# ZhendongS/Physics-Informed-Neural-Network-for-Explainable-Fault-Diagnosis-in-Fuel-Cells

Hardware: AMD Instinct MI355X
Metric: pinn_train_samples_per_s (higher is better)
Workload: dtype f32 (split-operand matrix products on the 16-bit matrix cores, f32 accumulate, fp32-matmul accuracy: 2 fp16 parts / 3 MFMAs per product in forward, backward and weight gradients); 1 GPU; BASELINE configs[1]: 1000000 synthetic rows x 8 features per GPU, PINN [8,256,256,256,1] + variance head, step = train_dnn (fwd+NLL+bwd+wgrad+allreduce+Adam) + one iteration of each of the 5 physics stages; rows_per_gpu=1000000, global_rows=1000000, parallelism=dp1, precision=f32x6, backend=none (single process), world_size=1

## Files before the change

### physics-informed-neural-network-for-explainable-fault-diagnosis-in-fuel-cells_amd/csrc/pinn_residuals.hip

```cpp
#include <hip/hip_runtime.h>
#include <math.h>
#include "../../include/pinn_hip.h"

namespace {

constexpr int kThreads = 256;
constexpr int kMaxBlocks = 1024;

struct AffineDev {
  double x_min[8];
  double x_scale[8];
  double y_min, y_scale;
  float vn_scale, vn_min;
};

__device__ __forceinline__ float denorm(float v, double mn, double sc) {
  float t = (float)((double)v - mn);
  return (float)((double)t / sc);
}

__device__ __forceinline__ float clamp_min_t(float x, float lo) { return x != x ? x : fmaxf(x, lo); }
__device__ __forceinline__ float clamp_t(float x, float lo, float hi) { return x != x ? x : fminf(fmaxf(x, lo), hi); }

__device__ __forceinline__ double wave_sum(double v) {
#pragma unroll
  for (int off = 32; off > 0; off >>= 1) v += __shfl_down(v, off, 64);
  return v;
}

struct LamDev {
  float l1, l2, l3, lT1, lT3, lT5, lH1, lH2, lH3, lO1, lO2, lO3, P_H2O;
};
__device__ __forceinline__ LamDev load_lambdas(const float* __restrict__ lambdas) {
  LamDev L;
  L.l1 = lambdas[PINN_L1]; L.l2 = lambdas[PINN_L2]; L.l3 = lambdas[PINN_L3];
  L.lT1 = lambdas[PINN_LT1]; L.lT3 = lambdas[PINN_LT3]; L.lT5 = lambdas[PINN_LT5];
  L.lH1 = lambdas[PINN_LH1]; L.lH2 = lambdas[PINN_LH2]; L.lH3 = lambdas[PINN_LH3];
  L.lO1 = lambdas[PINN_LO1]; L.lO2 = lambdas[PINN_LO2]; L.lO3 = lambdas[PINN_LO3];
  const float Tc = 55.0f;
  const float xw = ((-2.1794f + 0.02953f * Tc) - 9.1837e-5f * (Tc * Tc)) + 1.4454e-7f * ((Tc * Tc) * Tc);
  L.P_H2O = powf(10.0f, xw);
  return L;
}

template <bool kCols>
__device__ __forceinline__ void row_terms(long long row, const float* __restrict__ x, const float* __restrict__ u, const float* __restrict__ y,
                                          const AffineDev& aff, const LamDev& L, unsigned flags, float* __restrict__ cols, long long ld,
                                          float (&acc)[PINN_NSUMS]) {
  const float l1 = L.l1, l2 = L.l2, l3 = L.l3, lT1 = L.lT1, lT3 = L.lT3, lT5 = L.lT5, lH1 = L.lH1, lH2 = L.lH2, lH3 = L.lH3;
  const float lO1 = L.lO1, lO2 = L.lO2, lO3 = L.lO3, P_H2O = L.P_H2O;

    const float4 xa = reinterpret_cast<const float4*>(x)[row * 2];
    const float4 xb = reinterpret_cast<const float4*>(x)[row * 2 + 1];
    const bool fV = flags & PINN_RES_V, fT = flags & PINN_RES_T, fH = flags & PINN_RES_H, fO = flags & PINN_RES_O;
    const float r0 = denorm(xa.x, aff.x_min[0], aff.x_scale[0]);
    const float r1 = fT ? denorm(xa.y, aff.x_min[1], aff.x_scale[1]) : 0.f;
    const float r2 = fT ? denorm(xa.z, aff.x_min[2], aff.x_scale[2]) : 0.f;
    const float r3 = fV ? denorm(xa.w, aff.x_min[3], aff.x_scale[3]) : 0.f;
    const float r4 = fV ? denorm(xb.x, aff.x_min[4], aff.x_scale[4]) : 0.f;
    const float r5 = (fV || fT) ? denorm(xb.y, aff.x_min[5], aff.x_scale[5]) : 0.f;
    const float r6 = fH ? denorm(xb.z, aff.x_min[6], aff.x_scale[6]) : 0.f;
    const float r7 = fO ? denorm(xb.w, aff.x_min[7], aff.x_scale[7]) : 0.f;
    const float yv = (y != nullptr) ? y[row] : 0.0f;

    const float i5 = r0 / 270.0f + 1e-5f;
    const float It = i5 * 270.0f;

    if (flags & PINN_RES_V) {
      const float un = u[row];
      const float Tk = r5 + 273.15f;
      const float P_H2 = r3 / 101.0f + 1.0f;
      const float P_air = r4 / 101.0f + 1.0f;
      const float Tk_p = powf(Tk, 1.334f);
      const float pp_H2 = 0.5f * (P_H2 / expf(1.653f * i5 / Tk_p) - P_H2O);
      const float pp_O2 = P_air / expf(4.192f * i5 / Tk_p) - P_H2O;
      const float RT = 8.314f * Tk;
      const float b = RT / 96485.0f;
      const float V_act = (-b) * logf(i5 / l2);
      const float V_ohm = -(i5 * l1);
      const float V_conc = (0.5f * b) * logf(1.0f - i5 / l3);
      const float E = 220170.0f / 192970.0f - (RT * logf(P_H2O / (pp_H2 * sqrtf(pp_O2)))) / 192970.0f;
      const float V_est = ((E + V_act) + V_ohm) + V_conc;
      const float V_out = denorm(un, aff.y_min, aff.y_scale) / 5.0f;
      const float f = V_est - V_out;
// ... 25 lines not shown
        cols[PINN_C_I * ld + row] = i5;
        cols[PINN_C_VOUT5 * ld + row] = V_out * 5.0f;
      }
    }

    if (flags & PINN_RES_T) {
      const float i6 = r0 / 270.0f + 1e-6f;
      const float mc = r1 + 1e-6f;
      const float It6 = i6 * 270.0f;
      const float T_pred = ((lT1 * It6 + lT3 * mc) + 0.5f * r2) + lT5;
      const float f = r5 - T_pred;
      acc[PINN_S_FT2] += f * f;
      acc[PINN_S_FT_D1] += f * (-It6);
      acc[PINN_S_FT_D3] += f * (-mc);
      acc[PINN_S_FT_D5] += -f;
      acc[PINN_S_FT_ABS] += fabsf(f);
      if (kCols) {
        cols[PINN_C_FT * ld + row] = f;
        cols[PINN_C_TPRED * ld + row] = T_pred;
        cols[PINN_C_TOUT * ld + row] = r5;
      }
    }

    if (flags & PINN_RES_H) {
      float Q = ((It / 192970.0f) * 5.0f) * 22.4f;
      Q = Q * 60.0f;
      Q = clamp_min_t(Q, 1e-8f);
      const bool lin = It <= lH3;
      const float tgt = lin ? (lH1 + lH2 * (It / 100.0f)) : (lH1 + lH2 * (lH3 / 100.0f));
      const float act = (r6 + 1e-6f) / Q;
      const float f = act - tgt;
      acc[PINN_S_FH2] += f * f;
      acc[PINN_S_FH_D1] += -f;
      acc[PINN_S_FH_D2] += f * (-(lin ? It / 100.0f : lH3 / 100.0f));
      acc[PINN_S_FH_D3] += f * (-(lin ? 0.0f : lH2 / 100.0f));
      acc[PINN_S_ACTH] += act;
      acc[PINN_S_TGTH] += tgt;
      if (kCols) {
        cols[PINN_C_FH * ld + row] = f;
        cols[PINN_C_ACTH * ld + row] = act;
        cols[PINN_C_TGTH * ld + row] = tgt;
        cols[PINN_C_ITOT * ld + row] = It;
      }
    }

    if (flags & PINN_RES_O) {
      float Q = ((It * 5.0f) / 385940.0f) * 22.4f;
      Q = Q * 60.0f;
      Q = clamp_min_t(Q, 1e-8f);
      const float thr = fabsf(lO3);
      const bool lin = It <= thr;
      const float raw = lin ? (lO1 + lO2 * (It / 100.0f)) : (lO1 + lO2 * (thr / 100.0f));
      const float tgt = clamp_t(raw, 1.05f, 15.0f);
      const float c = (raw >= 1.05f && raw <= 15.0f) ? 1.0f : 0.0f;
      const float o2 = (r7 + 1e-6f) * 0.21f;
      const float act = o2 / Q;
      const float f = (act - tgt) + clamp_min_t(1.0f - act, 0.0f) * 10.0f;
      const float sgn = (lO3 > 0.0f) ? 1.0f : ((lO3 < 0.0f) ? -1.0f : 0.0f);
      acc[PINN_S_FO2] += f * f;
      acc[PINN_S_FO_D1] += f * (-c);
      acc[PINN_S_FO_D2] += f * (-c * (lin ? It / 100.0f : thr / 100.0f));
      acc[PINN_S_FO_D3] += f * (-c * (lin ? 0.0f : lO2 * sgn / 100.0f));
      acc[PINN_S_ACTO] += act;
      acc[PINN_S_TGTO] += tgt;
      if (kCols) {
        cols[PINN_C_FO * ld + row] = f;
        cols[PINN_C_ACTO * ld + row] = act;
        cols[PINN_C_TGTO * ld + row] = tgt;
        cols[PINN_C_QO2 * ld + row] = Q;
        cols[PINN_C_O2FLOW * ld + row] = o2;
      }
    }
  }

struct SumRange { int lo, hi; };
constexpr SumRange live_sums(unsigned flags) {
  return flags == PINN_RES_V ? SumRange{PINN_S_FV2, PINN_S_YU2 + 1}
       : flags == PINN_RES_T ? SumRange{PINN_S_FT2, PINN_S_FT_ABS + 1}
       : flags == PINN_RES_H ? SumRange{PINN_S_FH2, PINN_S_TGTH + 1}
       : flags == PINN_RES_O ? SumRange{PINN_S_FO2, PINN_S_TGTO + 1}
                             : SumRange{0, PINN_NSUMS};
}

template <int kLo, int kHi, int kBlock>
__device__ __forceinline__ void block_partials(const float (&acc)[PINN_NSUMS], double* __restrict__ partials) {
  __shared__ double red[kBlock / 64][kHi - kLo];
  const int lane = threadIdx.x & 63, wave = threadIdx.x >> 6;
#pragma unroll
  for (int s = kLo; s < kHi; ++s) {
    const double w = wave_sum((double)acc[s]);
    if (lane == 0) red[wave][s - kLo] = w;
  }
  __syncthreads();
  if (threadIdx.x < kHi - kLo) {
    double t = 0.0;
#pragma unroll
    for (int w = 0; w < kBlock / 64; ++w) t += red[w][threadIdx.x];
    partials[(long long)blockIdx.x * PINN_NSUMS + kLo + threadIdx.x] = t;
  }
}

template <bool kCols, unsigned kFlags>
__global__ __launch_bounds__(kThreads) void residuals_kernel(
    const float* __restrict__ x, const float* __restrict__ u, const float* __restrict__ y, AffineDev aff,
    const float* __restrict__ lambdas, unsigned flags_rt, long long n_rows, float* __restrict__ cols, long long ld,
    double* __restrict__ partials) {
  const unsigned flags = kFlags ? kFlags : flags_rt;
  const LamDev L = load_lambdas(lambdas);
  float acc[PINN_NSUMS];
#pragma unroll
  for (int s = 0; s < PINN_NSUMS; ++s) acc[s] = 0.0f;

  const long long stride = (long long)gridDim.x * kThreads;
  for (long long row = (long long)blockIdx.x * kThreads + threadIdx.x; row < n_rows; row += stride)
    row_terms<kCols>(row, x, u, y, aff, L, flags, cols, ld, acc);

  if (partials == nullptr) return;
  block_partials<live_sums(kFlags).lo, live_sums(kFlags).hi, kThreads>(acc, partials);
}

__global__ __launch_bounds__(1024) void residuals_finalize(const double* __restrict__ partials, int n_blocks, int s_lo, int s_hi,
                                                           double* __restrict__ sums) {
  __shared__ double red[32][PINN_NSUMS + 1];
  const int s = threadIdx.x & 31, j = threadIdx.x >> 5;
  if (s >= s_lo && s < s_hi) {
    double v[kMaxBlocks / 32];
#pragma unroll
    for (int k = 0; k < kMaxBlocks / 32; ++k) {
      const int b = j + 32 * k;
      v[k] = b < n_blocks ? partials[(long long)b * PINN_NSUMS + s] : 0.0;
    }
    double t = 0.0;
#pragma unroll
    for (int k = 0; k < kMaxBlocks / 32; ++k) t += v[k];
    red[j][s] = t;
  }
  __syncthreads();
  if (threadIdx.x < PINN_NSUMS) {
    double r = 0.0;
    if (threadIdx.x >= s_lo && threadIdx.x < s_hi) {
#pragma unroll
      for (int k = 0; k < 32; ++k) r += red[k][threadIdx.x];
    }
    sums[threadIdx.x] = r;
  }
}

struct StageDef {
  int n;
  int idx[5];
  float lo[5], hi[5];
};

__device__ __forceinline__ void lambda_step_body(int stage, const double* sums, double inv_n, float vn_scale, float lr, double bc1, double bc2, float* lambdas,
                                 float* adam, float* loss_out) {
  StageDef d;
  float g[5];
  bool has_grad[5];
  float total = 0.f, physics = 0.f;
  if (stage == PINN_STAGE_LAMBDA_PM || stage == PINN_STAGE_LAMBDA_F) {
    d.n = 4;
    d.idx[0] = PINN_L1; d.idx[1] = PINN_L2; d.idx[2] = PINN_L3; d.idx[3] = PINN_L4;
    d.lo[0] = (float)(0.167 * 0.5); d.hi[0] = (float)(0.167 * 5);
    d.lo[1] = (float)(2.36e-6 * 0.1); d.hi[1] = (float)(2.36e-6 * 2.1);
    d.lo[2] = 2.0f; d.hi[2] = (float)(2.0 * 5.2);
    d.lo[3] = 0.1f; d.hi[3] = 10.0f;
    has_grad[3] = false; g[3] = 0.f;
    if (stage == PINN_STAGE_LAMBDA_F) {
      physics = (float)(sums[PINN_S_FV2] * inv_n);
      for (int k = 0; k < 3; ++k) { g[k] = (float)(2.0 * sums[PINN_S_FV_D1 + k] * inv_n); has_grad[k] = true; }
    } else {
      physics = (float)(sums[PINN_S_YV2] * inv_n);
      for (int k = 0; k < 3; ++k) {
        g[k] = (float)(-2.0 * 5.0 * (double)vn_scale * sums[PINN_S_YV_D1 + k] * inv_n);
        has_grad[k] = true;
      }
    }
    total = physics + (float)(sums[PINN_S_YU2] * inv_n);
  } else if (stage == PINN_STAGE_THERMAL) {
    d.n = 5;
    for (int k = 0; k < 5; ++k) { d.idx[k] = PINN_LT1 + k; d.lo[k] = -10000.f; d.hi[k] = 10000.f; has_grad[k] = false; g[k] = 0.f; }
    g[0] = (float)(2.0 * sums[PINN_S_FT_D1] * inv_n); has_grad[0] = true;
    g[2] = (float)(2.0 * sums[PINN_S_FT_D3] * inv_n); has_grad[2] = true;
    g[4] = (float)(2.0 * sums[PINN_S_FT_D5] * inv_n); has_grad[4] = true;
    total = physics = (float)(sums[PINN_S_FT2] * inv_n);
  } else if (stage == PINN_STAGE_HYDROGEN) {
    d.n = 4;
    for (int k = 0; k < 4; ++k) d.idx[k] = PINN_LH1 + k;
    d.lo[0] = 0.5f; d.hi[0] = 50.f; d.lo[1] = -20.f; d.hi[1] = 20.f; d.lo[2] = 50.f; d.hi[2] = 1000.f; d.lo[3] = 0.f; d.hi[3] = 20.f;
    for (int k = 0; k < 3; ++k) { g[k] = (float)(2.0 * sums[PINN_S_FH_D1 + k] * inv_n); has_grad[k] = true; }
    has_grad[3] = false; g[3] = 0.f;
    total = physics = (float)(sums[PINN_S_FH2] * inv_n);
  } else {
    d.n = 4;
    for (int k = 0; k < 4; ++k) d.idx[k] = PINN_LO1 + k;
    d.lo[0] = 1.5f; d.hi[0] = 8.f; d.lo[1] = -20.f; d.hi[1] = 20.f; d.lo[2] = 50.f; d.hi[2] = 1000.f; d.lo[3] = 0.f; d.hi[3] = 20.f;
    for (int k = 0; k < 3; ++k) { g[k] = (float)(2.0 * sums[PINN_S_FO_D1 + k] * inv_n); has_grad[k] = true; }
    has_grad[3] = false; g[3] = 0.f;
    total = physics = (float)(sums[PINN_S_FO2] * inv_n);
  }
  const float step_size = (float)((double)lr / bc1);
  const float bc2_sqrt = (float)sqrt(bc2);
#pragma unroll
  for (int k = 0; k < 5; ++k) {
    if (k >= d.n) break;
    const int id = d.idx[k];
    float p = lambdas[id];
    if (has_grad[k]) {
      float m = adam[id], v = adam[PINN_NLAMBDA + id];
      m = m * 0.9f + g[k] * 0.1f;
      v = v * 0.999f + (g[k] * g[k]) * 0.001f;
      const float denom = sqrtf(v) / bc2_sqrt + 1e-8f;
      p = p - step_size * (m / denom);
      adam[id] = m; adam[PINN_NLAMBDA + id] = v;
    }
    lambdas[id] = clamp_t(p, d.lo[k], d.hi[k]);
  }
  if (loss_out) { loss_out[0] = total; loss_out[1] = physics; }
}

__global__ void lambda_step_kernel(int stage, const double* __restrict__ sums, double inv_n, float vn_scale, float lr,
                                   int step, float* __restrict__ lambdas, float* __restrict__ adam,
                                   float* __restrict__ loss_out) {
  if (threadIdx.x != 0 || blockIdx.x != 0) return;
  lambda_step_body(stage, sums, inv_n, vn_scale, lr, 1.0 - pow(0.9, (double)step), 1.0 - pow(0.999, (double)step), lambdas, adam, loss_out);
}

constexpr int kStageThreads = 1024;
// ... 133 lines not shown
      stage_prepare(row, x, u, y, aff, L0.P_H2O, flags, c);
#pragma unroll
      for (int k = 0; k < kCacheFloats; ++k) work[k * n_rows + row] = c[k];
    }
  }
  __syncthreads();
  constexpr int n_cached = cached_floats(kFlags);
  const double inv_n = 1.0 / (double)n_rows;
  double b1p = pow(0.9, (double)first_epoch), b2p = pow(0.999, (double)first_epoch);
  float lr = (float)(lr0 * pow(gamma, (double)(first_epoch / lr_step)));
  for (int it = 0; it < n_iters; ++it) {
    const int epoch = first_epoch + it;
    const LamDev L = load_lambdas(lam_s);
    float acc[PINN_NSUMS];
#pragma unroll
    for (int s = 0; s < PINN_NSUMS; ++s) acc[s] = 0.0f;
    constexpr int kTrip = (kFlags & PINN_RES_V) ? 2 : 4;
    for (long long row0 = tid; row0 < n_rows; row0 += kTrip * kStageThreads) {
      float c[kTrip][kCacheFloats];
#pragma unroll
      for (int q = 0; q < kTrip; ++q) {
        const long long row = row0 + q * kStageThreads;
        const long long rr = row < n_rows ? row : row0;
#pragma unroll
        for (int k = 0; k < kCacheFloats; ++k) c[q][k] = k < n_cached ? work[k * n_rows + rr] : 0.0f;
      }
#pragma unroll
      for (int q = 0; q < kTrip; ++q)
        if (row0 + q * kStageThreads < n_rows) stage_terms(c[q], aff, L, flags, acc);
    }
#pragma unroll
    for (int s = 0; s < PINN_NSUMS; ++s) {
      if (s >= s_lo && s < s_hi) {
        const double w = wave_sum((double)acc[s]);
        if (lane == 0) red[wave][s] = w;
      }
    }
    __syncthreads();
    if (tid >= s_lo && tid < s_hi) {
      double t = 0.0;
#pragma unroll
      for (int w = 0; w < kStageThreads / 64; ++w) t += red[w][tid];
      sums[tid] = t;
    }
    __syncthreads();
    if (tid == 0) {
      if (it > 0 && epoch % lr_step == 0) lr = (float)(lr0 * pow(gamma, (double)(epoch / lr_step)));
      b1p *= 0.9; b2p *= 0.999;
      lambda_step_body(stage, sums, inv_n, aff.vn_scale, lr, 1.0 - b1p, 1.0 - b2p, lam_s, adam_s, loss_s);
      if (log && log_every > 0 && epoch % log_every == 0) {
        float* row = log + (long long)(epoch / log_every - first_epoch / log_every) * kLogFloats;
        row[0] = loss_s[0]; row[1] = loss_s[1];
        row[2] = (float)(lr0 * pow(gamma, (double)((epoch + 1) / lr_step)));
        for (int k = 0; k < PINN_NLAMBDA; ++k) row[3 + k] = lam_s[k];
        for (int k = 0; k < PINN_NSUMS; ++k) row[20 + k] = (float)sums[k];
      }
    }
    __syncthreads();
  }
  if (tid < PINN_NLAMBDA) lambdas[tid] = lam_s[tid];
  if (tid < 2 * PINN_NLAMBDA) adam[tid] = adam_s[tid];
  if (tid < 2 && loss_out) loss_out[tid] = loss_s[tid];
  if (tid < PINN_NSUMS && sums_out) sums_out[tid] = sums[tid];
}


__global__ __launch_bounds__(kThreads) void stage_prepare_kernel(const float* __restrict__ x, const float* __restrict__ u,
                                                                 const float* __restrict__ y, AffineDev aff,
                                                                 const float* __restrict__ lambdas, unsigned flags, long long n_rows,
                                                                 float* __restrict__ cache) {
  const LamDev L0 = load_lambdas(lambdas);
  const long long stride = (long long)gridDim.x * kThreads;
  for (long long row = (long long)blockIdx.x * kThreads + threadIdx.x; row < n_rows; row += stride) {
    float c[kCacheFloats];
    stage_prepare(row, x, u, y, aff, L0.P_H2O, flags, c);
#pragma unroll
    for (int k = 0; k < kCacheFloats; ++k) cache[k * n_rows + row] = c[k];
  }
}

template <unsigned kFlags>
__global__ __launch_bounds__(kThreads) void residuals_cached_kernel(const float* __restrict__ cache, AffineDev aff,
                                                                    const float* __restrict__ lambdas, long long n_rows,
                                                                    double* __restrict__ partials) {
  const LamDev L = load_lambdas(lambdas);
  constexpr int n_cached = cached_floats(kFlags);
  float acc[PINN_NSUMS];
#pragma unroll
  for (int s = 0; s < PINN_NSUMS; ++s) acc[s] = 0.0f;
  const long long stride = (long long)gridDim.x * kThreads;
  for (long long row0 = (long long)blockIdx.x * kThreads + threadIdx.x; row0 < n_rows; row0 += 2 * stride) {
    float c[2][kCacheFloats];
#pragma unroll
    for (int q = 0; q < 2; ++q) {
      const long long row = row0 + q * stride;
      const long long rr = row < n_rows ? row : row0;
#pragma unroll
      for (int k = 0; k < kCacheFloats; ++k) c[q][k] = k < n_cached ? cache[k * n_rows + rr] : 0.0f;
    }
#pragma unroll
    for (int q = 0; q < 2; ++q)
      if (row0 + q * stride < n_rows) stage_terms(c[q], aff, L, kFlags, acc);
  }
  block_partials<live_sums(kFlags).lo, live_sums(kFlags).hi, kThreads>(acc, partials);
}

static AffineDev affine_dev(const pinn_affine_t* aff) {
  AffineDev a;
  for (int c = 0; c < 8; ++c) { a.x_min[c] = aff->x_min[c]; a.x_scale[c] = aff->x_scale[c]; }
  a.y_min = aff->y_min; a.y_scale = aff->y_scale; a.vn_scale = aff->vn_scale; a.vn_min = aff->vn_min;
  return a;
}
static int row_blocks(long long n_rows) {
  const long long want = (n_rows + kThreads - 1) / kThreads;
  return (int)(want < 1 ? 1 : (want > kMaxBlocks ? kMaxBlocks : want));
}
static bool one_stage_flag(unsigned flags) { return flags == PINN_RES_V || flags == PINN_RES_T || flags == PINN_RES_H || flags == PINN_RES_O; }


__global__ __launch_bounds__(kThreads) void net_f_T_kernel(const float* __restrict__ x, const float* __restrict__ u,
                                                           const float* __restrict__ x_halo, const float* __restrict__ u_halo, AffineDev aff,
                                                           const float* __restrict__ lambdas, long long n_rows, float* __restrict__ f_out,
                                                           float* __restrict__ t_pred, float* __restrict__ t_real) {
  const float lT1 = lambdas[PINN_LT1], lT2 = lambdas[PINN_LT2], lT3 = lambdas[PINN_LT3], lT4 = lambdas[PINN_LT4];
  for (long long row = (long long)blockIdx.x * blockDim.x + threadIdx.x; row < n_rows; row += (long long)gridDim.x * blockDim.x) {
    const float T_out = denorm(x[row * 8 + 5], aff.x_min[5], aff.x_scale[5]);
    float pred = T_out;
    const float* xp = row > 0 ? x + (row - 1) * 8 : x_halo;
    if (xp != nullptr) {
      const float4 pa = reinterpret_cast<const float4*>(xp)[0];
      const float4 pb = reinterpret_cast<const float4*>(xp)[1];
      const float un = row > 0 ? u[row - 1] : u_halo[0];
      const float r0 = denorm(pa.x, aff.x_min[0], aff.x_scale[0]);
      const float m_cool = denorm(pa.y, aff.x_min[1], aff.x_scale[1]) + 1e-6f;
      const float T_in = denorm(pa.z, aff.x_min[2], aff.x_scale[2]);
      const float T_prev = denorm(pb.y, aff.x_min[5], aff.x_scale[5]);
      const float i5 = r0 / 270.0f + 0.00001f;
      const float I_tot = i5 * 270.0f;
      const float Tk = T_prev + 273.15f;
      const float V_rev = 1.229f - 0.0009f * (Tk - 298.15f);
      const float V_cell = denorm(un, aff.y_min, aff.y_scale) / 5.0f;
      const float Q_el = (I_tot * V_rev - I_tot * V_cell) * lT4;
      const float Q_cool = ((m_cool * 4180.0f) * (T_prev - T_in)) * lT1;
      const float Q_rad = ((20.0f * 0.2f) * (T_prev - 25.0f)) * lT3;
      const float dT = ((Q_el - Q_cool) - Q_rad) / lT2;
      pred = T_prev + dT * 0.1f;
    }
    f_out[row] = T_out - pred;
    t_pred[row] = pred;
    t_real[row] = T_out;
  }
}

#define PINN_BIT(c) (1u << (c))
constexpr unsigned kGradColsV = PINN_BIT(PINN_C_FV) | PINN_BIT(PINN_C_VACT) | PINN_BIT(PINN_C_VOHM) | PINN_BIT(PINN_C_VCONC) |
                                PINN_BIT(PINN_C_ENERNST) | PINN_BIT(PINN_C_VEST5) | PINN_BIT(PINN_C_I) | PINN_BIT(PINN_C_VOUT5);
constexpr unsigned kGradColsT = PINN_BIT(PINN_C_FT) | PINN_BIT(PINN_C_TPRED) | PINN_BIT(PINN_C_TOUT);
constexpr unsigned kGradColsH = PINN_BIT(PINN_C_FH) | PINN_BIT(PINN_C_ACTH) | PINN_BIT(PINN_C_TGTH) | PINN_BIT(PINN_C_ITOT);
constexpr unsigned kGradColsO = PINN_BIT(PINN_C_FO) | PINN_BIT(PINN_C_ACTO) | PINN_BIT(PINN_C_TGTO) | PINN_BIT(PINN_C_QO2) |
                                PINN_BIT(PINN_C_O2FLOW);

__host__ __device__ inline unsigned grad_cols_of(unsigned flags) {
  return ((flags & PINN_RES_V) ? kGradColsV : 0u) | ((flags & PINN_RES_T) ? kGradColsT : 0u) | ((flags & PINN_RES_H) ? kGradColsH : 0u) |
         ((flags & PINN_RES_O) ? kGradColsO : 0u);
}

__device__ __forceinline__ void row_backward(long long row, const float* __restrict__ x, const float* __restrict__ u, const AffineDev& aff,
                                             const LamDev& L, unsigned flags, const float* __restrict__ g, long long ld, unsigned gmask,
                                             double (&acc)[PINN_NLAMBDA], float (&gr)[8], float& gu) {
  const float4 xa = reinterpret_cast<const float4*>(x)[row * 2];
  const float4 xb = reinterpret_cast<const float4*>(x)[row * 2 + 1];
  const bool fV = flags & PINN_RES_V, fT = flags & PINN_RES_T, fH = flags & PINN_RES_H, fO = flags & PINN_RES_O;
  const float r0 = denorm(xa.x, aff.x_min[0], aff.x_scale[0]);
  const float r1 = fT ? denorm(xa.y, aff.x_min[1], aff.x_scale[1]) : 0.f;
  const float r2 = fT ? denorm(xa.z, aff.x_min[2], aff.x_scale[2]) : 0.f;
  const float r3 = fV ? denorm(xa.w, aff.x_min[3], aff.x_scale[3]) : 0.f;
  const float r4 = fV ? denorm(xb.x, aff.x_min[4], aff.x_scale[4]) : 0.f;
  const float r5 = (fV || fT) ? denorm(xb.y, aff.x_min[5], aff.x_scale[5]) : 0.f;
  const float r6 = fH ? denorm(xb.z, aff.x_min[6], aff.x_scale[6]) : 0.f;
  const float r7 = fO ? denorm(xb.w, aff.x_min[7], aff.x_scale[7]) : 0.f;
#pragma unroll
  for (int c = 0; c < 8; ++c) gr[c] = 0.0f;
  gu = 0.0f;
  auto G = [&](int c) -> float { return (gmask & PINN_BIT(c)) ? g[(long long)c * ld + row] : 0.0f; };
  auto has = [&](unsigned bits) -> bool { return (gmask & bits) != 0u; };

  const float i5 = r0 / 270.0f + 1e-5f;
  const float It = i5 * 270.0f;
  float gi5 = 0.0f;

  if (fV) {
    const float gFV = G(PINN_C_FV), gVest = gFV + G(PINN_C_VEST5) * 5.0f;
    const float l1 = L.l1, l2 = L.l2, l3 = L.l3;
    float gi = G(PINN_C_I), gb = 0.0f, gTk = 0.0f;
    const float Tk = r5 + 273.15f;
    const float RT = 8.314f * Tk;
    const float b = RT / 96485.0f;
    if (has(PINN_BIT(PINN_C_FV) | PINN_BIT(PINN_C_VEST5) | PINN_BIT(PINN_C_VACT))) {
      const float gA = gVest + G(PINN_C_VACT);
      const float q = i5 / l2, La = logf(q);
// ... 233 lines not shown
  const float gdTc = gB * (m_cool * 4180.0f);
  gTp += gdTc;
  const float gC = -gnum * lT3;
  acc[PINN_LT3] += (double)(-gnum * C);
  gTp += gC * (20.0f * 0.2f);
  EulerGrad e;
  e.g0 = (gI * 270.0f) / 270.0f;
  e.g1 = (gB * dTc) * 4180.0f;
  e.g2 = -gdTc;
  e.g5 = gTp;
  e.gu = (float)((double)(gVcell / 5.0f) / aff.y_scale);
  return e;
}

__global__ __launch_bounds__(kThreads) void net_f_T_backward_kernel(
    const float* __restrict__ x, const float* __restrict__ u, const float* __restrict__ x_halo, const float* __restrict__ u_halo, AffineDev aff,
    const float* __restrict__ lambdas, long long n_rows, const float* __restrict__ gf, const float* __restrict__ gpred,
    const float* __restrict__ greal, float* __restrict__ gu_out, float* __restrict__ gx_out, float* __restrict__ gx_halo,
    float* __restrict__ gu_halo, double* __restrict__ partials) {
  __shared__ double red[kThreads / 64][PINN_NLAMBDA];
  const float lT1 = lambdas[PINN_LT1], lT2 = lambdas[PINN_LT2], lT3 = lambdas[PINN_LT3], lT4 = lambdas[PINN_LT4];
  double acc[PINN_NLAMBDA];
#pragma unroll
  for (int k = 0; k < PINN_NLAMBDA; ++k) acc[k] = 0.0;
  const bool step_path = gf != nullptr || gpred != nullptr;
  auto gp_at = [&](long long t) -> float { return (gpred ? gpred[t] : 0.0f) - (gf ? gf[t] : 0.0f); };
  const long long stride = (long long)gridDim.x * kThreads;
  for (long long row = (long long)blockIdx.x * kThreads + threadIdx.x; row < n_rows; row += stride) {
    float gr[8];
#pragma unroll
    for (int c = 0; c < 8; ++c) gr[c] = 0.0f;
    float gu = 0.0f;
    gr[5] = (gf ? gf[row] : 0.0f) + (greal ? greal[row] : 0.0f);
    if (row == 0 && x_halo == nullptr && step_path) gr[5] += gp_at(0);
    const float4 pa = reinterpret_cast<const float4*>(x)[row * 2];
    const float4 pb = reinterpret_cast<const float4*>(x)[row * 2 + 1];
    if (row + 1 < n_rows && step_path) {
      const EulerGrad e = euler_step_backward(pa, pb, u[row], gp_at(row + 1), aff, lT1, lT2, lT3, lT4, acc);
      gr[0] += e.g0; gr[1] += e.g1; gr[2] += e.g2; gr[5] += e.g5;
      gu = e.gu;
    }
    if (gx_out != nullptr) store_gx_row(gx_out, row, gr, aff);
    if (gu_out != nullptr) gu_out[row] = gu;
  }
  if (blockIdx.x == 0 && threadIdx.x == 0 && (gx_halo != nullptr || gu_halo != nullptr || x_halo != nullptr)) {
    float hr[8];
#pragma unroll
    for (int c = 0; c < 8; ++c) hr[c] = 0.0f;
    float hu = 0.0f;
    if (x_halo != nullptr && n_rows > 0 && step_path) {
      const float4 pa = reinterpret_cast<const float4*>(x_halo)[0];
      const float4 pb = reinterpret_cast<const float4*>(x_halo)[1];
      const EulerGrad e = euler_step_backward(pa, pb, u_halo[0], gp_at(0), aff, lT1, lT2, lT3, lT4, acc);
      hr[0] = e.g0; hr[1] = e.g1; hr[2] = e.g2; hr[5] = e.g5;
      hu = e.gu;
    }
    if (gx_halo != nullptr) store_gx_row(gx_halo, 0, hr, aff);
    if (gu_halo != nullptr) gu_halo[0] = hu;
  }
  block_lambda_partials(acc, red, partials);
}

}

extern "C" size_t pinn_residuals_workspace_bytes(void) { return (size_t)kMaxBlocks * PINN_NSUMS * sizeof(double); }

extern "C" int pinn_residuals(const float* d_x, const float* d_u, const float* d_y, const pinn_affine_t* aff,
                              const float* d_lambda, unsigned flags, long long n_rows, float* d_cols, long long ld,
                              double* d_sums, void* d_work, size_t work_bytes, void* stream) {
  if ((!d_x && n_rows > 0) || !aff || !d_lambda || n_rows < 0 || (flags & ~PINN_RES_ALL)) return PINN_E_ARG;
  if ((flags & PINN_RES_V) && !d_u && n_rows > 0) return PINN_E_ARG;
  if (d_cols && ld < n_rows) return PINN_E_ARG;
  if (d_sums && !d_work) return PINN_E_ARG;
  if (d_sums && work_bytes < pinn_residuals_workspace_bytes()) return PINN_E_WORKSPACE;
  hipStream_t st = (hipStream_t)stream;
  (void)hipGetLastError();
  AffineDev a;
  for (int c = 0; c < 8; ++c) { a.x_min[c] = aff->x_min[c]; a.x_scale[c] = aff->x_scale[c]; }
  a.y_min = aff->y_min; a.y_scale = aff->y_scale; a.vn_scale = aff->vn_scale; a.vn_min = aff->vn_min;
  long long want = (n_rows + kThreads - 1) / kThreads;
  int blocks = (int)(want < 1 ? 1 : (want > kMaxBlocks ? kMaxBlocks : want));
  double* partials = d_sums ? (double*)d_work : nullptr;
  const unsigned kf = (!d_cols && one_stage_flag(flags)) ? flags : 0u;
  if (n_rows > 0 || d_sums) {
#define PINN_RES_LAUNCH(COLS, F)                                                                                                  \
  hipLaunchKernelGGL((residuals_kernel<COLS, F>), dim3(blocks), dim3(kThreads), 0, st, d_x, d_u, d_y, a, d_lambda, flags, n_rows, \
                     d_cols, ld, partials)
    switch (kf) {
      case PINN_RES_V: PINN_RES_LAUNCH(false, PINN_RES_V); break;
      case PINN_RES_T: PINN_RES_LAUNCH(false, PINN_RES_T); break;
      case PINN_RES_H: PINN_RES_LAUNCH(false, PINN_RES_H); break;
      case PINN_RES_O: PINN_RES_LAUNCH(false, PINN_RES_O); break;
      default:
        if (d_cols) PINN_RES_LAUNCH(true, 0u);
        else PINN_RES_LAUNCH(false, 0u);
    }
#undef PINN_RES_LAUNCH
  }
  if (d_sums) {
    const SumRange live = live_sums(kf);
    hipLaunchKernelGGL(residuals_finalize, dim3(1), dim3(1024), 0, st, partials, blocks, live.lo, live.hi, d_sums);
  }
  hipError_t e = hipGetLastError();
  return e == hipSuccess ? PINN_OK : (int)e;
}

extern "C" int pinn_lambda_step(int stage, const double* d_sums, long long n_global, float vn_scale, float lr, int step,
                                float* d_lambda, float* d_adam, float* d_loss, void* stream) {
  if (stage < 0 || stage > PINN_STAGE_OXYGEN || !d_sums || n_global <= 0 || step < 1 || !d_lambda || !d_adam)
    return PINN_E_ARG;
  (void)hipGetLastError();
  hipLaunchKernelGGL(lambda_step_kernel, dim3(1), dim3(64), 0, (hipStream_t)stream, stage, d_sums, 1.0 / (double)n_global,
                     vn_scale, lr, step, d_lambda, d_adam, d_loss);
  hipError_t e = hipGetLastError();
  return e == hipSuccess ? PINN_OK : (int)e;
}

extern "C" size_t pinn_lambda_stage_workspace_bytes(long long n_rows) { return n_rows > 0 ? (size_t)n_rows * 6 * sizeof(float) : 0; }

extern "C" int pinn_lambda_stage_run(int stage, unsigned flags, const float* d_x, const float* d_u, const float* d_y, const pinn_affine_t* aff,
                                     long long n_rows, double lr0, double gamma, int lr_step, int first_epoch, int n_iters, float* d_lambda,
                                     float* d_adam, float* d_loss, float* d_log, int log_every, double* d_sums, void* d_work, size_t work_bytes,
                                     void* stream) {
  if (stage < 0 || stage > PINN_STAGE_OXYGEN || !d_x || !aff || !d_lambda || !d_adam || n_rows <= 0 || n_rows > PINN_STAGE_RUN_MAX_ROWS ||
      n_iters < 0 || first_epoch < 0 || lr_step < 1)
    return PINN_E_ARG;
  if (flags != PINN_RES_V && flags != PINN_RES_T && flags != PINN_RES_H && flags != PINN_RES_O) return PINN_E_ARG;
  if ((flags & PINN_RES_V) && (!d_u || !d_y)) return PINN_E_ARG;
  if (d_log && log_every > 0 && first_epoch % log_every) return PINN_E_ARG;
  if (!d_work) return PINN_E_ARG;
  if (work_bytes < pinn_lambda_stage_workspace_bytes(n_rows)) return PINN_E_WORKSPACE;
  if (n_iters == 0) return PINN_OK;
  (void)hipGetLastError();
  AffineDev a;
  for (int c = 0; c < 8; ++c) { a.x_min[c] = aff->x_min[c]; a.x_scale[c] = aff->x_scale[c]; }
  a.y_min = aff->y_min; a.y_scale = aff->y_scale; a.vn_scale = aff->vn_scale; a.vn_min = aff->vn_min;
#define PINN_STAGE_LAUNCH(F)                                                                                                          \
  hipLaunchKernelGGL((stage_run_kernel<F>), dim3(1), dim3(kStageThreads), 0, (hipStream_t)stream, stage, d_x, d_u, d_y, a, n_rows, lr0, gamma, \
                     lr_step, first_epoch, n_iters, d_lambda, d_adam, d_loss, d_log, log_every, d_sums, (float*)d_work)
  if (flags == PINN_RES_V) PINN_STAGE_LAUNCH(PINN_RES_V);
  else if (flags == PINN_RES_T) PINN_STAGE_LAUNCH(PINN_RES_T);
  else if (flags == PINN_RES_H) PINN_STAGE_LAUNCH(PINN_RES_H);
  else PINN_STAGE_LAUNCH(PINN_RES_O);
#undef PINN_STAGE_LAUNCH
  hipError_t e = hipGetLastError();
  return e == hipSuccess ? PINN_OK : (int)e;
}

extern "C" int pinn_residuals_prepare(const float* d_x, const float* d_u, const float* d_y, const pinn_affine_t* aff,
                                      const float* d_lambda, unsigned flags, long long n_rows, float* d_cache, void* stream) {
  if (!d_x || !aff || !d_lambda || !d_cache || n_rows <= 0 || !one_stage_flag(flags)) return PINN_E_ARG;
  if ((flags & PINN_RES_V) && (!d_u || !d_y)) return PINN_E_ARG;
  (void)hipGetLastError();
  hipLaunchKernelGGL(stage_prepare_kernel, dim3(row_blocks(n_rows)), dim3(kThreads), 0, (hipStream_t)stream, d_x, d_u, d_y, affine_dev(aff),
                     d_lambda, flags, n_rows, d_cache);
  hipError_t e = hipGetLastError();
  return e == hipSuccess ? PINN_OK : (int)e;
}

extern "C" int pinn_residuals_cached(const float* d_cache, const pinn_affine_t* aff, const float* d_lambda, unsigned flags,
                                     long long n_rows, double* d_sums, void* d_work, size_t work_bytes, void* stream) {
  if (!d_cache || !aff || !d_lambda || !d_sums || n_rows <= 0 || !one_stage_flag(flags)) return PINN_E_ARG;
  if (!d_work) return PINN_E_ARG;
  if (work_bytes < pinn_residuals_workspace_bytes()) return PINN_E_WORKSPACE;
  (void)hipGetLastError();
  hipStream_t st = (hipStream_t)stream;
  const int blocks = row_blocks((n_rows + 1) / 2);
#define PINN_CACHED_LAUNCH(F)                                                                                                     \
  hipLaunchKernelGGL((residuals_cached_kernel<F>), dim3(blocks), dim3(kThreads), 0, st, d_cache, affine_dev(aff), d_lambda, n_rows, \
                     (double*)d_work)
  if (flags == PINN_RES_V) PINN_CACHED_LAUNCH(PINN_RES_V);
  else if (flags == PINN_RES_T) PINN_CACHED_LAUNCH(PINN_RES_T);
  else if (flags == PINN_RES_H) PINN_CACHED_LAUNCH(PINN_RES_H);
  else PINN_CACHED_LAUNCH(PINN_RES_O);
#undef PINN_CACHED_LAUNCH
  const SumRange live = live_sums(flags);
  hipLaunchKernelGGL(residuals_finalize, dim3(1), dim3(1024), 0, st, (const double*)d_work, blocks, live.lo, live.hi, d_sums);
  hipError_t e = hipGetLastError();
  return e == hipSuccess ? PINN_OK : (int)e;
}

extern "C" int pinn_net_f_t(const float* d_x, const float* d_u, const float* d_x_halo, const float* d_u_halo, const pinn_affine_t* aff,
                            const float* d_lambda, long long n_rows, float* d_f, float* d_t_pred, float* d_t_real, void* stream) {
  if (n_rows < 0 || !aff || !d_lambda || (n_rows > 0 && (!d_x || !d_f || !d_t_pred || !d_t_real))) return PINN_E_ARG;
  if (n_rows > 1 && !d_u) return PINN_E_ARG;
  if ((d_x_halo == nullptr) != (d_u_halo == nullptr)) return PINN_E_ARG;
  if (n_rows == 0) return PINN_OK;
  (void)hipGetLastError();
  AffineDev a;
  for (int c = 0; c < 8; ++c) { a.x_min[c] = aff->x_min[c]; a.x_scale[c] = aff->x_scale[c]; }
  a.y_min = aff->y_min; a.y_scale = aff->y_scale; a.vn_scale = aff->vn_scale; a.vn_min = aff->vn_min;
  long long want = (n_rows + kThreads - 1) / kThreads;
  const int blocks = (int)(want > kMaxBlocks ? kMaxBlocks : want);
  hipLaunchKernelGGL(net_f_T_kernel, dim3(blocks), dim3(kThreads), 0, (hipStream_t)stream, d_x, d_u, d_x_halo, d_u_halo, a, d_lambda, n_rows,
                     d_f, d_t_pred, d_t_real);
  hipError_t e = hipGetLastError();
  return e == hipSuccess ? PINN_OK : (int)e;
}

static bool misaligned16(const void* p) { return ((unsigned long long)(size_t)p & 15ull) != 0ull; }

extern "C" int pinn_residuals_backward(const float* d_x, const float* d_u, const pinn_affine_t* aff, const float* d_lambda, unsigned flags,
                                       long long n_rows, const float* d_g, long long ld, unsigned gmask, float* d_glambda, float* d_gu,
                                       float* d_gx, void* d_work, size_t work_bytes, void* stream) {
  if (n_rows < 0 || !aff || !d_lambda || !d_glambda || (flags & ~PINN_RES_ALL)) return PINN_E_ARG;
  if (gmask & ~grad_cols_of(flags)) return PINN_E_ARG;
  if (n_rows > 0 && (!d_x || misaligned16(d_x) || misaligned16(d_gx))) return PINN_E_ARG;
  if ((flags & PINN_RES_V) && n_rows > 0 && !d_u) return PINN_E_ARG;
  if (gmask && n_rows > 0 && (!d_g || ld < n_rows)) return PINN_E_ARG;
  if (!d_work) return PINN_E_ARG;
  if (work_bytes < pinn_residuals_workspace_bytes()) return PINN_E_WORKSPACE;
  hipStream_t st = (hipStream_t)stream;
  (void)hipGetLastError();
  const int blocks = row_blocks(n_rows);
  hipLaunchKernelGGL(residuals_backward_kernel, dim3(blocks), dim3(kThreads), 0, st, d_x, d_u, affine_dev(aff), d_lambda, flags, n_rows,
                     d_g, ld, gmask, d_gu, d_gx, (double*)d_work);
  hipLaunchKernelGGL(lambda_grad_finalize, dim3(1), dim3(1024), 0, st, (const double*)d_work, blocks, d_glambda);
  hipError_t e = hipGetLastError();
  return e == hipSuccess ? PINN_OK : (int)e;
}

extern "C" int pinn_net_f_t_backward(const float* d_x, const float* d_u, const float* d_x_halo, const float* d_u_halo,
                                     const pinn_affine_t* aff, const float* d_lambda, long long n_rows, const float* d_gf,
                                     const float* d_gt_pred, const float* d_gt_real, float* d_glambda, float* d_gu, float* d_gx,
                                     float* d_gx_halo, float* d_gu_halo, void* d_work, size_t work_bytes, void* stream) {
  if (n_rows < 0 || !aff || !d_lambda || !d_glambda) return PINN_E_ARG;
  if (n_rows > 0 && (!d_x || misaligned16(d_x) || misaligned16(d_gx))) return PINN_E_ARG;
  if (n_rows > 1 && !d_u) return PINN_E_ARG;
  if ((d_x_halo == nullptr) != (d_u_halo == nullptr) || misaligned16(d_x_halo) || misaligned16(d_gx_halo)) return PINN_E_ARG;
  if (!d_x_halo && (d_gx_halo || d_gu_halo)) return PINN_E_ARG;
  if (!d_work) return PINN_E_ARG;
  if (work_bytes < pinn_residuals_workspace_bytes()) return PINN_E_WORKSPACE;
  hipStream_t st = (hipStream_t)stream;
  (void)hipGetLastError();
  const int blocks = row_blocks(n_rows);
  hipLaunchKernelGGL(net_f_T_backward_kernel, dim3(blocks), dim3(kThreads), 0, st, d_x, d_u, d_x_halo, d_u_halo, affine_dev(aff), d_lambda,
                     n_rows, d_gf, d_gt_pred, d_gt_real, d_gu, d_gx, d_gx_halo, d_gu_halo, (double*)d_work);
  hipLaunchKernelGGL(lambda_grad_finalize, dim3(1), dim3(1024), 0, st, (const double*)d_work, blocks, d_glambda);
  hipError_t e = hipGetLastError();
  return e == hipSuccess ? PINN_OK : (int)e;
}
```

Baseline: 233.2 million samples/s.

## Fuse residual finalize into last-block reduction via two-level atomic tickets

Replaces the separate single-block finalize launch after each residual kernel with a last-block-done pattern. Each block publishes its partial sums, then draws a two-level atomic ticket, and the final block reduces all partials into the sums. Ticket slots are assigned per stream, with a fallback to the old two-launch path for graph capture, the per-thread stream or slot exhaustion. This removes one kernel launch and its gap per residual call, at the cost of atomics, an acquire fence and a serialized tail reduction on one block.

```diff
diff --git a/physics-informed-neural-network-for-explainable-fault-diagnosis-in-fuel-cells_amd/csrc/pinn_residuals.hip b/physics-informed-neural-network-for-explainable-fault-diagnosis-in-fuel-cells_amd/csrc/pinn_residuals.hip
--- a/physics-informed-neural-network-for-explainable-fault-diagnosis-in-fuel-cells_amd/csrc/pinn_residuals.hip
+++ b/physics-informed-neural-network-for-explainable-fault-diagnosis-in-fuel-cells_amd/csrc/pinn_residuals.hip
@@ -1,5 +1,7 @@
 #include <hip/hip_runtime.h>
 #include <math.h>
+#include <stdlib.h>
+#include <mutex>
 #include "../../include/pinn_hip.h"
 
 namespace {
@@ -191,9 +193,48 @@
                              : SumRange{0, PINN_NSUMS};
 }
 
+template <int kBlock>
+__device__ __forceinline__ void reduce_partials(const double* partials, int n_blocks, int s_lo, int s_hi, double* sums,
+                                                double (*red)[PINN_NSUMS + 1]) {
+  const int n_live = s_hi - s_lo;
+#pragma unroll 1
+  for (int p = threadIdx.x; p < 32 * n_live; p += kBlock) {
+    const int j = p / n_live, s = s_lo + (p - j * n_live);
+    double v[kMaxBlocks / 32];
+#pragma unroll
+    for (int k = 0; k < kMaxBlocks / 32; ++k) {
+      const int b = j + 32 * k;
+      const double x = partials[(long long)(b < n_blocks ? b : 0) * PINN_NSUMS + s];
+      v[k] = b < n_blocks ? x : 0.0;
+    }
+    double t = 0.0;
+#pragma unroll
+    for (int k = 0; k < kMaxBlocks / 32; ++k) t += v[k];
+    red[j][s] = t;
+  }
+  __syncthreads();
+  if (threadIdx.x < PINN_NSUMS) {
+    double r = 0.0;
+    if (threadIdx.x >= s_lo && threadIdx.x < s_hi) {
+#pragma unroll
+      for (int k = 0; k < 32; ++k) r += red[k][threadIdx.x];
+    }
+    sums[threadIdx.x] = r;
+  }
+}
+
+constexpr int kTicketSlots = 32;
+constexpr int kTicketFan = 32;
+constexpr int kTicketStride = 64;
+static_assert(kTicketFan * kTicketFan >= kMaxBlocks, "two levels cover the grid cap");
+__device__ unsigned g_tickets[kTicketSlots][kTicketFan + 1][kTicketStride];
+
 template <int kLo, int kHi, int kBlock>
-__device__ __forceinline__ void block_partials(const float (&acc)[PINN_NSUMS], double* __restrict__ partials) {
+__device__ __forceinline__ void block_partials(const float (&acc)[PINN_NSUMS], double* partials, int ticket, double* sums) {
+  static_assert(kHi - kLo <= 64, "one wave stores the partial row and draws the ticket");
   __shared__ double red[kBlock / 64][kHi - kLo];
+  __shared__ double red_all[32][PINN_NSUMS + 1];
+  __shared__ unsigned last;
   const int lane = threadIdx.x & 63, wave = threadIdx.x >> 6;
 #pragma unroll
   for (int s = kLo; s < kHi; ++s) {
@@ -205,15 +246,37 @@
     double t = 0.0;
 #pragma unroll
     for (int w = 0; w < kBlock / 64; ++w) t += red[w][threadIdx.x];
-    partials[(long long)blockIdx.x * PINN_NSUMS + kLo + threadIdx.x] = t;
-  }
+    __hip_atomic_store(reinterpret_cast<long long*>(partials) + (long long)blockIdx.x * PINN_NSUMS + kLo + threadIdx.x, __double_as_longlong(t),
+                       __ATOMIC_RELAXED, __HIP_MEMORY_SCOPE_AGENT);
+  }
+  if (ticket < 0) return;
+  asm volatile("s_waitcnt vmcnt(0)" ::: "memory");
+  if (threadIdx.x == 0) {
+    const unsigned grid = gridDim.x, g = blockIdx.x % kTicketFan;
+    unsigned* const word = &g_tickets[ticket][g][0];
+    bool is_last = __hip_atomic_fetch_add(word, 1u, __ATOMIC_RELAXED, __HIP_MEMORY_SCOPE_AGENT) == (grid - g + kTicketFan - 1) / kTicketFan - 1;
+    if (is_last) {
+      __hip_atomic_store(word, 0u, __ATOMIC_RELAXED, __HIP_MEMORY_SCOPE_AGENT);
+      unsigned* const top = &g_tickets[ticket][kTicketFan][0];
+      is_last = __hip_atomic_fetch_add(top, 1u, __ATOMIC_RELAXED, __HIP_MEMORY_SCOPE_AGENT) == (grid < kTicketFan ? grid : kTicketFan) - 1;
+      if (is_last) {
+        __hip_atomic_store(top, 0u, __ATOMIC_RELAXED, __HIP_MEMORY_SCOPE_AGENT);
+        __builtin_amdgcn_fence(__ATOMIC_ACQUIRE, "agent");
+        asm volatile("s_waitcnt vmcnt(0)" ::: "memory");
+      }
+    }
+    last = is_last;
+  }
+  __syncthreads();
+  if (!last) return;
+  reduce_partials<kBlock>(partials, (int)gridDim.x, kLo, kHi, sums, red_all);
 }
 
 template <bool kCols, unsigned kFlags>
 __global__ __launch_bounds__(kThreads) void residuals_kernel(
     const float* __restrict__ x, const float* __restrict__ u, const float* __restrict__ y, AffineDev aff,
     const float* __restrict__ lambdas, unsigned flags_rt, long long n_rows, float* __restrict__ cols, long long ld,
-    double* __restrict__ partials) {
+    double* partials, int ticket, double* sums) {
   const unsigned flags = kFlags ? kFlags : flags_rt;
   const LamDev L = load_lambdas(lambdas);
   float acc[PINN_NSUMS];
@@ -225,34 +288,13 @@
     row_terms<kCols>(row, x, u, y, aff, L, flags, cols, ld, acc);
 
   if (partials == nullptr) return;
-  block_partials<live_sums(kFlags).lo, live_sums(kFlags).hi, kThreads>(acc, partials);
+  block_partials<live_sums(kFlags).lo, live_sums(kFlags).hi, kThreads>(acc, partials, ticket, sums);
 }
 
 __global__ __launch_bounds__(1024) void residuals_finalize(const double* __restrict__ partials, int n_blocks, int s_lo, int s_hi,
                                                            double* __restrict__ sums) {
   __shared__ double red[32][PINN_NSUMS + 1];
-  const int s = threadIdx.x & 31, j = threadIdx.x >> 5;
-  if (s >= s_lo && s < s_hi) {
-    double v[kMaxBlocks / 32];
-#pragma unroll
-    for (int k = 0; k < kMaxBlocks / 32; ++k) {
-      const int b = j + 32 * k;
-      v[k] = b < n_blocks ? partials[(long long)b * PINN_NSUMS + s] : 0.0;
-    }
-    double t = 0.0;
-#pragma unroll
-    for (int k = 0; k < kMaxBlocks / 32; ++k) t += v[k];
-    red[j][s] = t;
-  }
-  __syncthreads();
-  if (threadIdx.x < PINN_NSUMS) {
-    double r = 0.0;
-    if (threadIdx.x >= s_lo && threadIdx.x < s_hi) {
-#pragma unroll
-      for (int k = 0; k < 32; ++k) r += red[k][threadIdx.x];
-    }
-    sums[threadIdx.x] = r;
-  }
+  reduce_partials<1024>(partials, n_blocks, s_lo, s_hi, sums, red);
 }
 
 struct StageDef {
@@ -552,7 +594,7 @@
 template <unsigned kFlags>
 __global__ __launch_bounds__(kThreads) void residuals_cached_kernel(const float* __restrict__ cache, AffineDev aff,
                                                                     const float* __restrict__ lambdas, long long n_rows,
-                                                                    double* __restrict__ partials) {
+                                                                    double* partials, int ticket, double* sums) {
   const LamDev L = load_lambdas(lambdas);
   constexpr int n_cached = cached_floats(kFlags);
   float acc[PINN_NSUMS];
@@ -572,7 +614,7 @@
     for (int q = 0; q < 2; ++q)
       if (row0 + q * stride < n_rows) stage_terms(c[q], aff, L, kFlags, acc);
   }
-  block_partials<live_sums(kFlags).lo, live_sums(kFlags).hi, kThreads>(acc, partials);
+  block_partials<live_sums(kFlags).lo, live_sums(kFlags).hi, kThreads>(acc, partials, ticket, sums);
 }
 
 static AffineDev affine_dev(const pinn_affine_t* aff) {
@@ -586,6 +628,29 @@
   return (int)(want < 1 ? 1 : (want > kMaxBlocks ? kMaxBlocks : want));
 }
 static bool one_stage_flag(unsigned flags) { return flags == PINN_RES_V || flags == PINN_RES_T || flags == PINN_RES_H || flags == PINN_RES_O; }
+
+static int ticket_slot(hipStream_t st) {
+#ifdef PINN_DEBUG_HOOKS
+  static const bool two_launches = getenv("PINN_RESIDUALS_TWO_LAUNCHES") != nullptr;
+  if (two_launches) return -1;
+#endif
+  if (st == hipStreamPerThread) return -1;
+  hipStreamCaptureStatus capture = hipStreamCaptureStatusNone;
+  if (hipStreamIsCapturing(st, &capture) != hipSuccess) {
+    (void)hipGetLastError();
+    return -1;
+  }
+  if (capture != hipStreamCaptureStatusNone) return -1;
+  static std::mutex mu;
+  static hipStream_t seen[kTicketSlots] = {nullptr};
+  static int n_seen = 1;
+  std::lock_guard<std::mutex> lock(mu);
+  for (int i = 0; i < n_seen; ++i)
+    if (seen[i] == st) return i;
+  if (n_seen == kTicketSlots) return -1;
+  seen[n_seen] = st;
+  return n_seen++;
+}
 
 
 __global__ __launch_bounds__(kThreads) void net_f_T_kernel(const float* __restrict__ x, const float* __restrict__ u,
@@ -985,10 +1050,11 @@
   int blocks = (int)(want < 1 ? 1 : (want > kMaxBlocks ? kMaxBlocks : want));
   double* partials = d_sums ? (double*)d_work : nullptr;
   const unsigned kf = (!d_cols && one_stage_flag(flags)) ? flags : 0u;
+  const int ticket = d_sums ? ticket_slot(st) : -1;
   if (n_rows > 0 || d_sums) {
 #define PINN_RES_LAUNCH(COLS, F)                                                                                                  \
   hipLaunchKernelGGL((residuals_kernel<COLS, F>), dim3(blocks), dim3(kThreads), 0, st, d_x, d_u, d_y, a, d_lambda, flags, n_rows, \
-                     d_cols, ld, partials)
+                     d_cols, ld, partials, ticket, d_sums)
     switch (kf) {
       case PINN_RES_V: PINN_RES_LAUNCH(false, PINN_RES_V); break;
       case PINN_RES_T: PINN_RES_LAUNCH(false, PINN_RES_T); break;
@@ -1000,7 +1066,7 @@
     }
 #undef PINN_RES_LAUNCH
   }
-  if (d_sums) {
+  if (d_sums && ticket < 0) {
     const SumRange live = live_sums(kf);
     hipLaunchKernelGGL(residuals_finalize, dim3(1), dim3(1024), 0, st, partials, blocks, live.lo, live.hi, d_sums);
   }
@@ -1069,16 +1135,19 @@
   (void)hipGetLastError();
   hipStream_t st = (hipStream_t)stream;
   const int blocks = row_blocks((n_rows + 1) / 2);
+  const int ticket = ticket_slot(st);
 #define PINN_CACHED_LAUNCH(F)                                                                                                     \
   hipLaunchKernelGGL((residuals_cached_kernel<F>), dim3(blocks), dim3(kThreads), 0, st, d_cache, affine_dev(aff), d_lambda, n_rows, \
-                     (double*)d_work)
+                     (double*)d_work, ticket, d_sums)
   if (flags == PINN_RES_V) PINN_CACHED_LAUNCH(PINN_RES_V);
   else if (flags == PINN_RES_T) PINN_CACHED_LAUNCH(PINN_RES_T);
   else if (flags == PINN_RES_H) PINN_CACHED_LAUNCH(PINN_RES_H);
   else PINN_CACHED_LAUNCH(PINN_RES_O);
 #undef PINN_CACHED_LAUNCH
-  const SumRange live = live_sums(flags);
-  hipLaunchKernelGGL(residuals_finalize, dim3(1), dim3(1024), 0, st, (const double*)d_work, blocks, live.lo, live.hi, d_sums);
+  if (ticket < 0) {
+    const SumRange live = live_sums(flags);
+    hipLaunchKernelGGL(residuals_finalize, dim3(1), dim3(1024), 0, st, (const double*)d_work, blocks, live.lo, live.hi, d_sums);
+  }
   hipError_t e = hipGetLastError();
   return e == hipSuccess ? PINN_OK : (int)e;
 }
```

Result: no change. 233.8 million samples/s (median of 6 runs) (+0.3%).
